# zhaobinglei/REGNet_for_3D_Grasping

Measured on AMD Instinct MI355X. Metric: scenes/sec (25 600-pt ScoreNet+GRN fwd), higher is better.
Workload: dtype f32; 1 GPU; configs[2]: ScoreNet+GraspRegionNet+RefineNet forward, 25600-pt synthetic scenes, batch=8 per GPU, eval; points=25600, batch_per_gpu=8, global_batch=8, parallelism=scene-sharded x1 (no data-path collective), sampling_group_batches=8, sampling_lookahead_batches=32, distinct_batches=8, region_head=synthetic.calibrate_region_head on batch 0, geometry_pending_at_enqueue=9, hip_graphs=False

## Files before the change

### include/regnet_hip.h

```cpp
#ifndef REGNET_HIP_H_
#define REGNET_HIP_H_

#include <stdint.h>

#ifdef __cplusplus
extern "C" {
#endif

#define REGNET_OK 0
#define REGNET_ERR_SHAPE (-1)
#define REGNET_ERR_NULL (-2)
#define REGNET_ERR_UNSUPPORTED (-3)

int regnet_abi_version(void);
const char* regnet_build_info(void);
const char* regnet_strerror(int code);

int regnet_fps_f32(const float* xyz, int64_t sb, int64_t sc, int64_t sn, int64_t B, int64_t N,
                   int64_t M, int64_t* index, float* workspace, void* stream);
int64_t regnet_fps_workspace_bytes(int64_t B, int64_t N, int64_t M);
int regnet_fps_chain_f32(const float* xyz, int64_t sb, int64_t sc, int64_t sn, int64_t B, int64_t N, int64_t M,
                         int64_t* index, float* workspace, const int32_t* prefix_ok, int32_t* first_tie, void* stream);
int64_t regnet_fps_status_offset_bytes(int64_t B, int64_t N, int64_t M);
int regnet_fps_plan(int64_t B, int64_t N, int64_t M, int64_t* plan);

int regnet_ball_query_f32(const float* xyz, int64_t sb, int64_t sc, int64_t sn,
                          const float* centroids, int64_t cb, int64_t cc, int64_t cn, int64_t B,
                          int64_t N1, int64_t N2, float radius, int64_t K, int64_t* index,
                          int64_t* count, void* stream);

int64_t regnet_grid_workspace_bytes(int64_t B, int64_t N_source);
int regnet_three_nn_grid_f32(const float* query, int64_t qb, int64_t qc, int64_t qn, const float* key,
                             int64_t kb, int64_t kc, int64_t kn, int64_t B, int64_t N1, int64_t N2,
                             int64_t* index, float* dist2, void* workspace, void* stream);
int regnet_ball_query_grid_f32(const float* xyz, int64_t sb, int64_t sc, int64_t sn,
                               const float* centroids, int64_t cb, int64_t cc, int64_t cn, int64_t B,
                               int64_t N1, int64_t N2, float radius, int64_t K, int64_t* index,
                               int64_t* count, void* workspace, void* stream);

int regnet_group_points_fwd_f32(const float* input, int64_t sb, int64_t sc, int64_t sn,
                                const int64_t* index, int64_t B, int64_t C, int64_t N1, int64_t N2,
                                int64_t K, float* out, void* stream);
int regnet_group_points_bwd_f32(const float* grad_out, int64_t sb, int64_t sc, int64_t sn2,
                                int64_t sk, const int64_t* index, int64_t B, int64_t C, int64_t N1,
                                int64_t N2, int64_t K, float* grad_in, void* stream);

int regnet_three_nn_f32(const float* query, int64_t qb, int64_t qc, int64_t qn, const float* key,
                        int64_t kb, int64_t kc, int64_t kn, int64_t B, int64_t N1, int64_t N2,
                        int64_t* index, float* dist2, void* stream);

int regnet_interpolate_fwd_f32(const float* input, int64_t sb, int64_t sc, int64_t sm,
                               const int64_t* index, const float* weight, int64_t B, int64_t C,
                               int64_t M, int64_t N, float* out, void* stream);
int regnet_interpolate_bwd_f32(const float* grad_out, int64_t sb, int64_t sc, int64_t sn,
                               const int64_t* index, const float* weight, int64_t B, int64_t C,
                               int64_t M, int64_t N, float* grad_in, void* stream);

int regnet_gather_knn_fwd_f32(const float* input, int64_t sb, int64_t sc, int64_t sn,
                              const int64_t* index, int64_t B, int64_t C, int64_t N, int64_t NI,
                              int64_t K, float* out, void* stream);
int regnet_gather_knn_bwd_f32(const float* grad_out, int64_t sb, int64_t sc, int64_t sn2,
                              int64_t sk, const int64_t* index, int64_t B, int64_t C, int64_t N,
                              int64_t NI, int64_t K, float* grad_in, void* stream);

int64_t regnet_fps_f64_workspace_bytes(int64_t B, int64_t N, int64_t M);
int regnet_fps_f64(const double* xyz, int64_t sb, int64_t sc, int64_t sn, int64_t B, int64_t N, int64_t M,
                   int64_t* index, double* workspace, void* stream);
int regnet_ball_query_f64(const double* xyz, int64_t sb, int64_t sc, int64_t sn, const double* centroids, int64_t cb,
                          int64_t cc, int64_t cn, int64_t B, int64_t N1, int64_t N2, float radius, int64_t K,
                          int64_t* index, int64_t* count, void* stream);
int regnet_three_nn_f64(const double* query, int64_t qb, int64_t qc, int64_t qn, const double* key, int64_t kb,
                        int64_t kc, int64_t kn, int64_t B, int64_t N1, int64_t N2, int64_t* index, double* dist2,
                        void* stream);
int64_t regnet_scatter_f64_workspace_bytes(int64_t B, int64_t num_dest, int64_t num_src);
int regnet_group_points_fwd_f64(const double* input, int64_t sb, int64_t sc, int64_t sn, const int64_t* index, int64_t B,
                                int64_t C, int64_t N1, int64_t N2, int64_t K, double* out, void* stream);
int regnet_group_points_bwd_f64(const double* grad_out, int64_t sb, int64_t sc, int64_t sn2, int64_t sk,
                                const int64_t* index, int64_t B, int64_t C, int64_t N1, int64_t N2, int64_t K,
                                double* grad_in, void* workspace, void* stream);
int regnet_interpolate_fwd_f64(const double* input, int64_t sb, int64_t sc, int64_t sm, const int64_t* index,
                               const double* weight, int64_t B, int64_t C, int64_t M, int64_t N, double* out,
                               void* stream);
int regnet_interpolate_bwd_f64(const double* grad_out, int64_t sb, int64_t sc, int64_t sn, const int64_t* index,
                               const double* weight, int64_t B, int64_t C, int64_t M, int64_t N, double* grad_in,
                               void* workspace, void* stream);
int regnet_gather_knn_fwd_f64(const double* input, int64_t sb, int64_t sc, int64_t sn, const int64_t* index, int64_t B,
                              int64_t C, int64_t N, int64_t NI, int64_t K, double* out, void* stream);
int regnet_gather_knn_bwd_f64(const double* grad_out, int64_t sb, int64_t sc, int64_t sn2, int64_t sk,
                              const int64_t* index, int64_t B, int64_t C, int64_t N, int64_t NI, int64_t K,
                              double* grad_in, void* workspace, void* stream);

int regnet_radius_group_f32(const float* pc, int64_t pb, int64_t pn, const float* centres,
                            int64_t cb, int64_t cn, int64_t B, int64_t N, int64_t NC,
                            float d2_threshold, int64_t cap, int32_t* cand, int32_t* count,
                            void* stream);

int regnet_select_positive_f32(const float* pc, int64_t pb, int64_t pn, const float* score, int64_t sb,
                               int64_t B, int64_t N, float threshold, int64_t* index, float* xyz_out,
                               int32_t* count, void* stream);

int regnet_box_crop_f32(const float* group_points, int64_t gb, int64_t gn, const float* centre,
                        const float* rot, const float* xlim, const float* ylim, float zlim,
                        int64_t n, int64_t G, int32_t* cand, int32_t* count, void* stream);

int regnet_gather_max_f32(const float* feat, int64_t num_rows, int64_t F, const int64_t* rows,
                          int64_t R, int64_t G, float* out, void* stream);
int regnet_gather_max_scene_f32(const float* feat, int64_t num_rows, int64_t F, const int64_t* rows, const int64_t* row_ids,
                                int64_t R, int64_t G, int64_t per_scene, int64_t scene_stride, float* out, void* stream);

int regnet_mlp_layer_f32(const float* A, int64_t lda, int64_t Ka, const float* W, int64_t Kpad,
                         const float* scale, const float* shift, float* C, int64_t ldc, int64_t P,
                         int64_t N, int relu, int pool_group, void* stream);

int64_t regnet_mlp_splitk_workspace_bytes(int64_t P, int64_t N, int64_t ksplit);
int regnet_mlp_layer_splitk_f32(const float* A, int64_t lda, int64_t Ka, const float* W, int64_t Kpad,
                                const float* scale, const float* shift, float* C, int64_t ldc, int64_t P,
                                int64_t N, int relu, int64_t ksplit, void* workspace, void* stream);

int regnet_mlp_layer_plan(int64_t P, int64_t N, int64_t Kpad, int pool_group, int64_t* plan);

int regnet_sa_layer1_f32(const float* feat, int64_t fb, int64_t fn, int64_t fc, int64_t Cf,
                         const float* xyz, int64_t xb, int64_t xc, int64_t xn, const int64_t* nbr,
                         const int64_t* ctr, int64_t B, int64_t M, int64_t group, const float* W,
                         int64_t Kpad, const float* scale, const float* shift, float* C, int64_t ldc,
                         int64_t N, int relu, void* stream);

int regnet_sa_layer12_f32(const float* feat, int64_t fb, int64_t fn, int64_t fc, int64_t Cf,
                          const float* xyz, int64_t xb, int64_t xc, int64_t xn, const int64_t* nbr,
// ... 339 lines not shown
```

### regnet_for_3d_grasping_amd/csrc/build.py

```python
import hashlib
import os
import subprocess
import sys

HERE = os.path.dirname(os.path.abspath(__file__))
OUT = os.path.join(HERE, "libregnet_hip.so")
ARCH = "gfx950"

SOURCES = [
    ("api.hip", []),
    ("geometry.hip", ["-ffp-contract=off", "-fno-slp-vectorize"]),
    ("gather.hip", []),
    ("region.hip", ["-ffp-contract=off"]),
    ("grid.hip", ["-ffp-contract=off"]),
    ("mlp.hip", []),
    ("sa_chain.hip", ["-fno-slp-vectorize"]),
    ("rowchain.hip", ["-fno-slp-vectorize"]),
    ("heads.hip", []),
    ("heads_train.hip", []),
    ("losses.hip", ["-ffp-contract=off"]),
    ("tgemm.hip", []),
    ("sa_split.hip", ["-fno-slp-vectorize"]),
    ("tsplit.hip", []),
    ("bn_train.hip", []),
# ... 10 lines not shown
    ("cluster.hip", ["-ffp-contract=off"]),
    ("fuse.hip", ["-ffp-contract=off"]),
    ("icp.hip", ["-ffp-contract=off"]),
    ("approach.hip", ["-ffp-contract=off"]),
    ("outlier.hip", ["-ffp-contract=off"]),
    ("tsdf.hip", ["-ffp-contract=off"]),
]
COMMON = ["--offload-arch=" + ARCH, "-O3", "-std=c++17", "-fPIC", "-Wall", "-Wno-unused-function",
          "-fno-gpu-rdc"]


def _hipcc():
    for cand in (os.environ.get("HIPCC"), "/opt/rocm/bin/hipcc", "hipcc"):
        if cand and (os.path.isabs(cand) and os.path.exists(cand) or not os.path.isabs(cand)):
            return cand
    raise RuntimeError("hipcc not found")


def _stamp():
    h = hashlib.sha256()
    for name in sorted(os.listdir(HERE)):
        if name.endswith((".hip", ".h", ".py")):
            with open(os.path.join(HERE, name), "rb") as f:
                h.update(name.encode()); h.update(f.read())
    inc = os.path.join(HERE, "..", "..", "include", "regnet_hip.h")
    with open(inc, "rb") as f:
        h.update(f.read())
    return h.hexdigest()


REPO = os.path.dirname(os.path.dirname(HERE))
NO_VGPR_SPILL = {"mlp.o": ["mlp_gemm_kernelILi0E", "gemm2_kernel"], "sa_chain.o": ["sa_chain_kernel"],
                 "rowchain.o": ["sa_premul_chain_kernel", "sa3_premul_chain_kernel", "fp_head_chain_kernelILb0E"],
                 "heads.o": ["heads_chain_kernel", "heads_tree_kernel"], "ops_f64.o": ["_f64_kernel"],
                 "scatter.o": ["scatter_", "segsum_"], "det.o": ["det_"],
                 "ingest.o": ["ingest_"], "nms.o": ["nms_"], "plane.o": ["plane_"], "depth.o": ["depth_"],
                 "fuse.o": ["fuse_"], "icp.o": ["icp_"], "outlier.o": ["outlier_"], "tsdf.o": ["tsdf_"]}


def check_no_vgpr_spill(obj_path, fragments):
    import shutil
    import tempfile
    llvm = "/opt/rocm/lib/llvm/bin"
    objdump, readelf = os.path.join(llvm, "llvm-objdump"), os.path.join(llvm, "llvm-readelf")
    if not (os.path.exists(objdump) and os.path.exists(readelf)):
        return None
    tmp = tempfile.mkdtemp(prefix="regnet_co_")
    try:
        local = os.path.join(tmp, os.path.basename(obj_path))
        shutil.copy(obj_path, local)
        subprocess.run([objdump, "--offloading", local], cwd=tmp, stdout=subprocess.DEVNULL, stderr=subprocess.DEVNULL)
        found = 0
        for name in os.listdir(tmp):
            if "amdgcn" not in name:
                continue
            notes = subprocess.run([readelf, "--notes", os.path.join(tmp, name)], stdout=subprocess.PIPE, stderr=subprocess.DEVNULL).stdout.decode()
            kernel = None
            for line in notes.splitlines():
                line = line.strip()
                if line.startswith(".name:"):
                    kernel = line.split(":", 1)[1].strip()
                elif line.startswith(".vgpr_spill_count:") and kernel and any(f in kernel for f in fragments):
                    found += 1
                    if int(line.split(":", 1)[1]) != 0:
                        raise RuntimeError("%s: %s spills %s vector registers" % (os.path.basename(obj_path), kernel, line.split(":", 1)[1].strip()))
        return found
# ... 78 lines not shown
```

### regnet_for_3d_grasping_amd/csrc/grid.hip

```cpp
#include "grid.h"

__device__ __forceinline__ void nn3_insert(float d, int j, float& d0, float& d1, float& d2, int& i0, int& i1,
                                           int& i2) {
  const bool b2 = d < d2 || (d == d2 && j < i2);
  if (!b2) return;
  const bool b1 = d < d1 || (d == d1 && j < i1);
  const bool b0 = d < d0 || (d == d0 && j < i0);
  d2 = b1 ? d1 : d;
  i2 = b1 ? i1 : j;
  d1 = b0 ? d0 : (b1 ? d : d1);
  i1 = b0 ? i0 : (b1 ? j : i1);
  d0 = b0 ? d : d0;
  i0 = b0 ? j : i0;
}

__global__ __launch_bounds__(256) void three_nn_grid_kernel(const float* __restrict__ query, int64_t qb, int64_t qc,
                                                            int64_t qn, int N1, const char* __restrict__ ws,
                                                            long long slab, int64_t* __restrict__ index,
                                                            float* __restrict__ dist2) {
  const int b = blockIdx.y;
  const int i = blockIdx.x * 256 + threadIdx.x;
  if (i >= N1) return;
  char* my = const_cast<char*>(ws) + (long long)b * slab;
  const GridHeader H = *reinterpret_cast<const GridHeader*>(my);
// ... 292 lines not shown
      }
    }
  }
  int m = 0;
  if (A[1][1] < A[m][m]) m = 1;
  if (A[2][2] < A[m][m]) m = 2;
  n[0] = m == 0 ? V[0][0] : (m == 1 ? V[0][1] : V[0][2]);
  n[1] = m == 0 ? V[1][0] : (m == 1 ? V[1][1] : V[1][2]);
  n[2] = m == 0 ? V[2][0] : (m == 1 ? V[2][1] : V[2][2]);
}

__global__ __launch_bounds__(256) void normal_eigen_kernel(const float* __restrict__ xyz, int N,
                                                           const double* __restrict__ cov, const int* __restrict__ count,
                                                           double cx, double cy, double cz, float* __restrict__ normals) {
  const int i = blockIdx.x * 256 + threadIdx.x;
  if (i >= N) return;
  double n[3] = {0., 0., 1.};
  if (count[i] >= 3) {
    sym3_min_eigenvector(cov + (int64_t)i * 6, n);
    if (n[0] == 0. && n[1] == 0. && n[2] == 0.) { n[2] = 1.; }
  }
  double len = sqrt(n[0] * n[0] + n[1] * n[1] + n[2] * n[2]);
  if (len > 0.) { n[0] /= len; n[1] /= len; n[2] /= len; }
  const double rx = cx - (double)xyz[(int64_t)i * 3], ry = cy - (double)xyz[(int64_t)i * 3 + 1],
               rz = cz - (double)xyz[(int64_t)i * 3 + 2];
  if (n[0] * rx + n[1] * ry + n[2] * rz < 0.) { n[0] = -n[0]; n[1] = -n[1]; n[2] = -n[2]; }
  normals[(int64_t)i * 3] = (float)n[0];
  normals[(int64_t)i * 3 + 1] = (float)n[1];
  normals[(int64_t)i * 3 + 2] = (float)n[2];
}

extern "C" int64_t regnet_grid_workspace_bytes(int64_t B, int64_t N) { return B * grid_slab_bytes(N); }

extern "C" int regnet_three_nn_grid_f32(const float* query, int64_t qb, int64_t qc, int64_t qn, const float* key,
                                        int64_t kb, int64_t kc, int64_t kn, int64_t B, int64_t N1, int64_t N2,
                                        int64_t* index, float* dist2, void* workspace, void* stream) {
  if (N2 < 3 || B < 0 || N1 < 0) return REGNET_ERR_SHAPE;
  if (N1 >= (int64_t)1 << 31 || N2 >= (int64_t)1 << 31 || B > 65535) return REGNET_ERR_UNSUPPORTED;
  if (B == 0 || N1 == 0) return REGNET_OK;
  if (!query || !key || !index || !dist2 || !workspace) return REGNET_ERR_NULL;
  hipStream_t st = as_stream(stream);
  int rc = build_grid(key, kb, kc, kn, B, N2, 0.f, workspace, st);
  if (rc) return rc;
  dim3 grid((unsigned)((N1 + 255) / 256), (unsigned)B);
  hipLaunchKernelGGL(three_nn_grid_kernel, grid, dim3(256), 0, st, query, qb, qc, qn, (int)N1, (const char*)workspace,
                     grid_slab_bytes(N2), index, dist2);
  REGNET_LAUNCH_CHECK();
  return REGNET_OK;
}

extern "C" int regnet_ball_query_grid_f32(const float* xyz, int64_t sb, int64_t sc, int64_t sn, const float* centroids,
                                          int64_t cb, int64_t cc, int64_t cn, int64_t B, int64_t N1, int64_t N2,
                                          float radius, int64_t K, int64_t* index, int64_t* count, void* workspace,
                                          void* stream) {
  if (K <= 0 || B < 0 || N1 < 0 || N2 < 0) return REGNET_ERR_SHAPE;
  if (K > 64 || !(radius > 0.f) || N1 >= (int64_t)1 << 31 || N2 >= (int64_t)1 << 31 || B > 65535)
    return REGNET_ERR_UNSUPPORTED;
  if (B == 0 || N2 == 0) return REGNET_OK;
  if (!centroids || !index || !count || !workspace || (N1 > 0 && !xyz)) return REGNET_ERR_NULL;
  hipStream_t st = as_stream(stream);
  int rc = build_grid(xyz, sb, sc, sn, B, N1, radius, workspace, st);
  if (rc) return rc;
  const float r2 = radius * radius;
  dim3 grid((unsigned)((N2 + 3) / 4), (unsigned)B);
  hipLaunchKernelGGL(ball_query_grid_kernel, grid, dim3(256), 0, st, centroids, cb, cc, cn, (int)N2, r2, radius, (int)K,
                     (const char*)workspace, grid_slab_bytes(N1), index, count);
// ... 31 lines not shown
```

### regnet_for_3d_grasping_amd/csrc/region.hip

```cpp
#include "common.h"

#define RG_WAVES 4

#define RG_UNROLL 4
__device__ __forceinline__ unsigned long long rg_hits(const float* __restrict__ p, int64_t pn, int j, int end,
                                                      float cx, float cy, float cz, float thr) {
  bool hit = false;
  if (j < end) {
    const float* r = p + (int64_t)j * pn;
    hit = sqdist3(r[0], r[1], r[2], cx, cy, cz) <= thr;
  }
  return __ballot(hit);
}

__global__ __launch_bounds__(RG_WAVES * 64) void radius_group_kernel(
    const float* __restrict__ pc, int64_t pb, int64_t pn, const float* __restrict__ ctr, int64_t cb, int64_t cn,
    int N, int NC, float thr, int64_t cap, int32_t* __restrict__ cand, int32_t* __restrict__ count) {
  __shared__ int wave_cnt[RG_WAVES];
  const int lane = threadIdx.x & 63, wave = threadIdx.x >> 6;
  const int c = blockIdx.x;
  const int b = blockIdx.y;
  const float* p = pc + (int64_t)b * pb;
  const float* q = ctr + (int64_t)b * cb + (int64_t)c * cn;
  const float cx = q[0], cy = q[1], cz = q[2];
  int32_t* out = cand + ((int64_t)b * NC + c) * cap;
  const unsigned long long lt_mask = (1ull << lane) - 1ull;
  const int per = ((N + RG_WAVES - 1) / RG_WAVES + 63) / 64 * 64;
  const int beg = min(N, wave * per), end = min(N, beg + per);
  int cnt = 0;
  for (int j0 = beg; j0 < end; j0 += 64 * RG_UNROLL) {
    unsigned long long m[RG_UNROLL];
#pragma unroll
    for (int u = 0; u < RG_UNROLL; ++u) m[u] = rg_hits(p, pn, j0 + 64 * u + lane, end, cx, cy, cz, thr);
#pragma unroll
    for (int u = 0; u < RG_UNROLL; ++u) cnt += (int)__popcll(m[u]);
  }
  if (lane == 0) wave_cnt[wave] = cnt;
  __syncthreads();
  int base = 0, total = 0;
#pragma unroll
  for (int w = 0; w < RG_WAVES; ++w) {
    const int v = wave_cnt[w];
    base += w < wave ? v : 0;
    total += v;
  }
  if (threadIdx.x == 0) count[(int64_t)b * NC + c] = total;
  if (cnt == 0 || base >= cap) return;
  for (int j0 = beg; j0 < end; j0 += 64 * RG_UNROLL) {
    unsigned long long m[RG_UNROLL];
#pragma unroll
    for (int u = 0; u < RG_UNROLL; ++u) m[u] = rg_hits(p, pn, j0 + 64 * u + lane, end, cx, cy, cz, thr);
#pragma unroll
    for (int u = 0; u < RG_UNROLL; ++u) {
      if ((m[u] >> lane) & 1ull) {
        const int pos = base + (int)__popcll(m[u] & lt_mask);
        if (pos < cap) out[pos] = j0 + 64 * u + lane;
      }
      base += (int)__popcll(m[u]);
    }
  }
}

extern "C" int regnet_radius_group_f32(const float* pc, int64_t pb, int64_t pn, const float* centres, int64_t cb,
                                       int64_t cn, int64_t B, int64_t N, int64_t NC, float d2_threshold,
                                       int64_t cap, int32_t* cand, int32_t* count, void* stream) {
  if (B < 0 || N < 0 || NC < 0 || cap < 0) return REGNET_ERR_SHAPE;
  if (N >= (int64_t)1 << 31 || B > 65535) return REGNET_ERR_UNSUPPORTED;
  if (B == 0 || NC == 0) return REGNET_OK;
  if (!centres || !count || (cap > 0 && !cand) || (N > 0 && !pc)) return REGNET_ERR_NULL;
  if (NC >= (int64_t)1 << 31) return REGNET_ERR_UNSUPPORTED;
  dim3 grid((unsigned)NC, (unsigned)B);
  hipLaunchKernelGGL(radius_group_kernel, grid, dim3(RG_WAVES * 64), 0, as_stream(stream), pc, pb, pn, centres, cb,
                     cn, (int)N, (int)NC, d2_threshold, cap, cand, count);
  REGNET_LAUNCH_CHECK();
  return REGNET_OK;
}

#define SP_WAVES 8
__global__ __launch_bounds__(SP_WAVES * 64) void select_positive_kernel(const float* __restrict__ pc, int64_t pb, int64_t pn,
                                                                       const float* __restrict__ score, int64_t sb, int N,
                                                                       float thr, int64_t* __restrict__ index,
                                                                       float* __restrict__ xyz_out, int32_t* __restrict__ count) {
  __shared__ int wave_cnt[SP_WAVES];
  const int tid = threadIdx.x, lane = tid & 63;
  const int wave = __builtin_amdgcn_readfirstlane(tid >> 6);
  const int b = blockIdx.x;
  const float* p = pc + (int64_t)b * pb;
  const float* sc = score + (int64_t)b * sb;
  int64_t* idx = index + (int64_t)b * N;
  float* xo = xyz_out + (int64_t)b * 3 * N;
  const unsigned long long lt_mask = (1ull << lane) - 1ull;
  const int seg = ((N + SP_WAVES - 1) / SP_WAVES + 63) / 64 * 64;
  const int lo = wave * seg, hi = lo + seg < N ? lo + seg : N;
// ... 610 lines not shown
```

### regnet_for_3d_grasping_amd/fused.py

```python
import collections
import ctypes

import torch

from . import _lib, pn2_ext

ENABLED = True
CHAIN3 = True
SPLITK_MAX_ROWS = 1024
PREMUL = True
PREMUL_CENTRE = True
ROWCHAIN = True
SA3_CHAIN = True
FP_HEAD_INTERP = True

SaRoute = collections.namedtuple("SaRoute", "features tail prepare")


def sa_route(module, has_feature=True):
    mlp, n = module.mlp, len(module.mlp)
    if getattr(module.grouper, "num_neighbours", 0) != 64 or n < 2 or (has_feature and not module.use_xyz):
        return None
    width = [block.conv.out_channels for block in mlp]
    relu = [block.relu is not None for block in mlp]
# ... 419 lines not shown
    "sa_layer1": lambda feature, xyz, nbr, ctr, layer, B, M, group: _flop_meta(B * M * group, layer.K, layer.N),
    "sa_premul_layer": lambda U, V, nbr, layer, B, Nsrc, M, group, pool_group=0:
        _flop_meta(B * M * group, layer.K, layer.N),
    "sa_chain3": lambda feature, xyz, nbr, ctr, l1, l2, l3, B, M, group, count=None, order=None:
        "P%d K%d N%d flop%d" % (B * M * group, l3.K, l3.N,
                                2 * B * M * group * (l1.K * l1.N + l2.K * l2.N + l3.K * l3.N)),
    "sa_premul_chain": lambda U, V, nbr, module, layers, B, Nsrc, M:
        "P%d K256 N512 flop%d" % (B * M * 64, 2 * B * M * 64 * (256 * 256 + 256 * 512)),
    "sa3_premul_chain": lambda U, V, nbr, module, layers, B, Nsrc, M:
        "P%d K512 N1024 flop%d" % (B * M * 64, 2 * B * M * 64 * (512 * 512 + 512 * 1024)),
    "fp_head_chain_interp": lambda Ys, idx, dist2, eps, dense_small, wd4, first, seg, fp_layers, B, Ns, Nd:
        "P%d K256 N256 flop%d" % (B * Nd, 2 * B * Nd * 491520),
    "fp_head_chain": lambda h1, seg, fp_layers, P: "P%d K256 N256 flop%d" % (P, 2 * P * 491520),
    "sa_layer12": lambda feature, xyz, nbr, ctr, first, layer, B, M, group, pool_group=0:
        "P%d K%d N%d flop%d" % (B * M * group, layer.K, layer.N,
                                2 * B * M * group * (layer.K * layer.N + first.K * first.N)),
}


def _as_channels_last(feature):
    cl = feature.transpose(1, 2)
    return cl if cl.is_contiguous() else cl.contiguous()


def sa_sample(module, xyz, prefix_ok=None):
    chain = pn2_ext.FpsChain(prefix_ok if FPS_CHAIN else None)
    ctr = pn2_ext.farthest_point_sample(xyz, module.num_centroids, chain)
    return ctr, chain.first_tie


def sa_group(module, xyz, ctr, first_tie=None):
    B, M = ctr.shape
    new_xyz = pn2_ext.gather_points(xyz, ctr) if xyz.dtype == torch.float32 else torch.gather(xyz, 2, ctr[:, None, :].expand(B, 3, M))
    nbr, count = pn2_ext.ball_query(xyz, new_xyz, module.grouper.radius, module.grouper.num_neighbours)
    geo = {"ctr": ctr, "new_xyz": new_xyz, "nbr": nbr}
    if first_tie is not None:
        geo["first_tie"] = first_tie
    route = sa_route(module)
    prepare = route.prepare if route is not None else None
    if prepare == "pairs":
        geo["count"] = count
        geo["order"] = chain3_pair_order(count)
    elif prepare == "premul":
        _, (_, v_layer) = _sa_packs(module, route, module.mlp[0].conv.in_channels - 3, xyz.device)
        geo.update(_premul_centres(xyz, new_xyz, v_layer))
    return geo


def sa_geometry(module, xyz, ctr=None, prefix_ok=None):
    if ctr is not None:
        return sa_group(module, xyz, ctr)
    ctr, first_tie = sa_sample(module, xyz, prefix_ok)
    return sa_group(module, xyz, ctr, first_tie)


def sa_features(module, xyz, feature, geo):
    B, N1 = xyz.shape[0], xyz.shape[2]
    M, K = module.num_centroids, module.grouper.num_neighbours
    Cf = 0 if feature is None else feature.size(1)
    route = sa_route(module, feature is not None)
    if route is None:
        raise NotImplementedError("fused SA supports 64 neighbours, >= 2 MLP layers and features only with use_xyz")
    layers, premul = _sa_packs(module, route, Cf, xyz.device)
    P = B * M * K
    pool = 0 if route.tail else K
    nbr, ctr = geo["nbr"], geo["ctr"]
    if premul is not None:
        u_layer, v_layer = premul
# ... 388 lines not shown
```

### regnet_for_3d_grasping_amd/get_regiondataset.py

```python
import numpy as np
import torch

from . import host_io, np_random, region_ops
from .pn2_utils import function as _F


def get_grasp_allobj(pc, predict_score, params, data_paths, use_theta=True, defer_large_groups=False):
    (center_num, score_thre, group_num, r_time_group, group_num_more, r_time_group_more,
     width, height, depth) = params
    center_pc, center_pc_index = _select_score_center(pc, predict_score, center_num, score_thre)
    labels_pending = None
    if pc.is_cuda and (DEVICE_DRAWS or (pc.shape[0] * pc.shape[1] > BATCHED_SEARCH_MAX_POINTS and len(data_paths) == 0)):
        pc_group_index, pc_group = _get_group_pc(pc, center_pc, center_pc_index, group_num, width, height, depth,
                                                 r_time_group)
        pc_group_more_index, pc_group_more = _get_group_pc(pc, center_pc, center_pc_index, group_num_more, width,
                                                           height, depth, r_time_group_more)
    else:
        cand_s, count_s = region_ops.radius_candidates(pc, center_pc, group_radius(width, height, depth, r_time_group))
        cand_m, count_m = region_ops.radius_candidates(pc, center_pc, group_radius(width, height, depth, r_time_group_more))
        if len(data_paths) > 0 and pc.is_cuda:
            labels_pending = _get_center_grasp(center_pc_index, center_pc, data_paths, depth, use_theta, defer_read=True)
        np_random.flush()
        counts = torch.stack((count_s, count_m)).cpu().numpy()
        def drawn(count, size):
            if pc.is_cuda:
                return np_random.choice_rows_pinned(count, size, 0)[0].to(pc.device, non_blocking=True)
            return host_io.upload(np_random.choice_rows(count, size, 0)[0], pc.device)

        pos = drawn(counts[0], group_num)
        pc_group_index, pc_group = region_ops.resample_groups(pc, cand_s, pos)

        def large_groups():
            return region_ops.resample_groups(pc, cand_m, drawn(counts[1], group_num_more))

        if defer_large_groups and DEFER_LARGE_GROUPS and pc.is_cuda:
            pc_group_more_index, pc_group_more = large_groups, None
        else:
            pc_group_more_index, pc_group_more = large_groups()
    grasp_labels = None
    if labels_pending is not None:
        grasp_labels = labels_pending() if callable(labels_pending) else labels_pending
    elif len(data_paths) > 0:
        grasp_labels = _get_center_grasp(center_pc_index, center_pc, data_paths, depth, use_theta)
    np_random.flush_unless_deferred()
    return center_pc, center_pc_index, pc_group_index, pc_group, pc_group_more_index, pc_group_more, grasp_labels


DEFER_LARGE_GROUPS = True
LABEL_KERNEL = True
BATCHED_LABELS = True
NO_GRASP_SQ_DISTANCE = 0.005

# ... 163 lines not shown
            np_random.flush()
            extra = np.random.choice(P, center_num - P, replace=True)
            local = torch.cat([torch.arange(P), torch.from_numpy(np.asarray(extra, dtype=np.int64))])
            index[b] = map_index[local.to(pc.device)]
        else:
            np_random.flush()
            picks = np.random.choice(N, center_num, replace=False)
            index[b] = host_io.upload(np.asarray(picks, dtype=np.int64), pc.device)
    if pc.is_cuda and pc.dtype == torch.float32:
        from . import pn2_ext
        center_pc = pn2_ext.gather_points(pc.transpose(1, 2), index, channels_last=True)
    else:
        center_pc = torch.gather(pc, 1, index.unsqueeze(-1).expand(B, center_num, C))
    return center_pc, index


def group_radius(width, height, depth, r_time):
    return float(np.float32(max(width, height, depth) * r_time))


DEVICE_DRAWS = False
BATCHED_SEARCH_MAX_POINTS = 4 * 25600


def _draw_positions(counts, group_num, max_count):
    if DEVICE_DRAWS and counts.is_cuda:
        return np_random.choice_rows_device(counts.int(), group_num, 0, max_count)[0]
    np_random.flush()
    if counts.is_cuda:
        return np_random.choice_rows_pinned(counts.cpu().numpy(), group_num, 0)[0].to(counts.device, non_blocking=True)
    return host_io.upload(np_random.choice_rows(counts.cpu().numpy(), group_num, 0)[0], counts.device)


def _get_group_pc(pc, center_pc, center_pc_index, group_num, width, height, depth, r_time):
    B, N, C = pc.shape
    Nc = center_pc.shape[1]
    radius = group_radius(width, height, depth, r_time)
    cand, counts = region_ops.radius_candidates(pc, center_pc, radius)
    pos = _draw_positions(counts, group_num, N)
    pc_group_index, pc_group = region_ops.resample_groups(pc, cand, pos)
    return pc_group_index, pc_group
```

### regnet_for_3d_grasping_amd/pipeline.py

```python
import contextlib
import io

import torch

from . import synthetic
from .get_regiondataset import get_grasp_allobj
from .gripper_region_network import GripperRegionNetwork
from .score_network import ScoreNetwork

CENTER_NUM, SCORE_THRE = 64, 0.5
GROUP_NUM, R_TIME_GROUP = 256, 0.1
GROUP_NUM_MORE, R_TIME_GROUP_MORE = 1024, 0.8
WIDTH, HEIGHT, DEPTH = 0.08, 0.01, 0.06
GRIPPER_NUM, GRASP_SCORE_THRESHOLD, REG_CHANNEL = 64, 0.5, 10

PARAMS = [CENTER_NUM, SCORE_THRE, GROUP_NUM, R_TIME_GROUP, GROUP_NUM_MORE, R_TIME_GROUP_MORE, WIDTH, HEIGHT, DEPTH]
GRIPPER_PARAMS = [WIDTH, HEIGHT, DEPTH]


def build_models(device, score_seed=7, region_seed=11):
    score_net = ScoreNetwork(training=True)
    score_net.load_state_dict(synthetic.seeded_state_dict(score_net, score_seed))
    region_net = GripperRegionNetwork(training=True, group_num=GROUP_NUM, gripper_num=GRIPPER_NUM,
                                      grasp_score_threshold=GRASP_SCORE_THRESHOLD, radius=DEPTH,
# ... 260 lines not shown
    def _wants_graphs(self, pc):
        want = self.graphs
        if want == "auto":
            want = pc.shape[0] * pc.shape[1] <= GRAPH_MAX_POINTS
        from . import fused
        return bool(want) and fused.ENABLED and len(self.s_mlps) == 1 and not self.score_net.training and pc.is_cuda

    def _features(self, item):
        if "slot" in item:
            return self._features_replay(item)
        s_mlp = self.s_mlps[self._n_featured % len(self.s_mlps)]
        self._n_featured += 1
        from . import fused
        prev = self.__dict__.get("_last_mlp_done")
        if prev is not None and prev.query():
            self.host_late_feature_stages = self.__dict__.get("host_late_feature_stages", 0) + 1
        geo_pending = not item["geo_done"].query()
        if geo_pending:
            self.geometry_pending_at_enqueue = self.__dict__.get("geometry_pending_at_enqueue", 0) + 1
        with torch.cuda.stream(s_mlp), torch.no_grad():
            s_mlp.wait_event(item["geo_done"])
            fused.TAIL_SINK = tails = [] if self.split_chain_tail else None
            try:
                all_feature, score, _ = self.score_net(item["pc"], plan=item["plan"])
            finally:
                fused.TAIL_SINK = None
            done = torch.cuda.Event()
            done.record(s_mlp)
            self._last_mlp_done = done
            item["tail_done"] = list(tails or ())
        all_feature.record_stream(self.s_reg)
        score.record_stream(self.s_reg)
        item.update(all_feature=all_feature, score=score, mlp_done=done)
        item.pop("plan")
        item.pop("ctr")
        return item

    def _region(self, item):
        pc, all_feature, score = item["pc"], item["all_feature"], item["score"]
        out = {"all_feature": all_feature, "score": score}
        with torch.cuda.stream(self.s_reg), torch.no_grad():
            self.s_reg.wait_event(item["mlp_done"])
            for ev in item.get("tail_done", ()):
                self.s_reg.wait_event(ev)
            if self.with_region:
                (center_pc, center_idx, g_idx, g, gm_idx, gm, _) = get_grasp_allobj(pc, score, PARAMS, [])
                with contextlib.redirect_stdout(io.StringIO()):
                    res = self.region_net(g, gm, g_idx, gm_idx, center_pc, center_idx, pc, all_feature,
                                          GRIPPER_PARAMS, None, [])
                out.update(center_pc_index=center_idx, pc_group_index=g_idx, pc_group_more_index=gm_idx,
                           next_grasp=res[0], keep_per_scene=res[1], true_mask=res[2], select_grasp_class=res[6],
                           select_grasp_score=res[7], final_mask=res[11],
                           valid_crops=getattr(self.region_net, "last_valid_crops", None))
            done = torch.cuda.Event()
            done.record(self.s_reg)
        if not self.with_region:
            item["mlp_done"].synchronize()
            for ev in item.get("tail_done", ()):
                ev.synchronize()
        out["done"] = done
        return out

    def run(self, batches, max_pending_regions=3):
        import queue
        import threading

        from . import fused
        cur = torch.cuda.current_stream(self.device)
        with torch.no_grad():
            fused.prepack(self.score_net, self.region_net)
        self._graph_sig = _graph_signature(self.score_net)
        if self._stage_graphs is not None and self._stage_graphs.signature != self._graph_sig:
            self._stage_graphs = None
        streams = tuple(self.s_fps) + tuple(self.s_mlps) + (self.s_geo, self.s_reg)
        for s in streams:
            s.wait_stream(cur)

        todo, done = queue.Queue(), queue.Queue()

# ... 101 lines not shown
```

### regnet_for_3d_grasping_amd/pn2_ext.py

```python
import torch

from . import _lib, determinism

_call = _lib.call
_L = _lib.lib

GRID_MIN_POINTS = 2048
GRID_MIN_POINTS_BALL = 8192


def _need_gpu(t, name):
    if not isinstance(t, torch.Tensor):
        raise TypeError("%s must be a torch.Tensor" % name)
    if not t.is_cuda:
        raise RuntimeError("%s must be a CUDA tensor" % name)


def _need_f32(t, name):
    _need_gpu(t, name)
    if t.dtype != torch.float32:
        raise RuntimeError("%s must be float32 (REGNet's path is fp32 only)" % name)


def _need_float(t, name, like=None):
    _need_gpu(t, name)
    if t.dtype not in (torch.float32, torch.float64):
        raise RuntimeError("%s must be float32 or float64" % name)
    if like is not None and t.dtype != like.dtype:
        raise RuntimeError("%s is %s but the other float inputs are %s" % (name, t.dtype, like.dtype))
    return t.dtype == torch.float64


# ... 81 lines not shown
    _call("regnet_class_order_i64", count, flat.data_ptr(), flat.numel(), order.data_ptr())
    return order


def pair_order(count):
    _need_i64(count, "count")
    flat = count.reshape(-1)
    flat = flat if flat.is_contiguous() else flat.contiguous()
    order = torch.empty((flat.numel(),), dtype=torch.int64, device=count.device)
    work = torch.empty((flat.numel(),), dtype=torch.int32, device=count.device)
    _call("regnet_pair_order_i64", count, flat.data_ptr(), flat.numel(), order.data_ptr(), work.data_ptr())
    return order


_fps_flags = {}


def _fps_flag(device):
    key = (device.type, device.index if device.index is not None else torch.cuda.current_device())
    if key not in _fps_flags:
        _fps_flags[key] = torch.zeros(1, dtype=torch.int32, device=device)
    return _fps_flags[key]


def raise_if_fps_failed():
    for flag in _fps_flags.values():
        if int(flag.item()):
            flag.zero_()
            raise RuntimeError("farthest_point_sample: a cooperating workgroup lost its partner (launch not fully "
                               "resident?) -- the returned indices are incomplete -- or gather_points saw an index "
                               "outside the cloud")


def ball_query(points, centroids, radius, num_neighbours):
    f64 = _need_float(points, "points")
    _need_float(centroids, "centroids", points)
    _eq(points.size(1), 3, "points.size(1) does not equal to 3")
    _eq(centroids.size(1), 3, "centroids.size(1) does not equal to 3")
    _eq(centroids.size(0), points.size(0), "centroids.size(0) does not equal to batch_size")
    B, _, N1 = points.shape
    N2 = centroids.size(2)
    K = int(num_neighbours)
    index = torch.empty((B, N2, K), dtype=torch.int64, device=points.device)
    count = torch.empty((B, N2), dtype=torch.int64, device=points.device)
    if not f64 and N1 >= GRID_MIN_POINTS_BALL and K <= 64 and B > 0 and float(radius) > 0:
        ws = torch.empty((_L.regnet_grid_workspace_bytes(B, N1),), dtype=torch.uint8, device=points.device)
        _call("regnet_ball_query_grid_f32", points, points.data_ptr(), *points.stride(), centroids.data_ptr(),
              *centroids.stride(), B, N1, N2, float(radius), K, index.data_ptr(), count.data_ptr(), ws.data_ptr())
    else:
        _call(_entry("ball_query", points), points, points.data_ptr(), *points.stride(), centroids.data_ptr(),
              *centroids.stride(), B, N1, N2, float(radius), K, index.data_ptr(), count.data_ptr())
    return [index, count]


def group_points_forward(input, index):
    _need_float(input, "input")
    _need_i64(index, "index")
    _eq(input.dim(), 3, "input.dim() does not equal to 3")
    _eq(index.dim(), 3, "index.dim() does not equal to 3")
    _eq(index.size(0), input.size(0), "index.size(0) does not equal to batch_size")
    B, C, N1 = input.shape
    _, N2, K = index.shape
    idx = index.contiguous()
    out = torch.empty((B, C, N2, K), dtype=input.dtype, device=input.device)
    _call(_entry("group_points_fwd", input), input, input.data_ptr(), *input.stride(), idx.data_ptr(), B, C, N1, N2, K,
          out.data_ptr())
    return out


def group_points_backward(grad_output, index, num_points, plan=None):
    _need_float(grad_output, "grad_output")
    _need_i64(index, "index")
    _eq(grad_output.dim(), 4, "grad_output.dim() does not equal to 4")
    _eq(index.dim(), 3, "index.dim() does not equal to 3")
    B, C, N2, K = grad_output.shape
    _eq(index.size(0), B, "index.size(0) does not equal to batch_size")
    _eq(index.size(1), N2, "index.size(1) does not equal to num_select")
    _eq(index.size(2), K, "index.size(2) does not equal to k")
    N1 = int(num_points)
    idx = index.contiguous()
    return _scatter_backward(
# ... 115 lines not shown
```

### regnet_for_3d_grasping_amd/region_ops.py

```python
import numpy as np
import torch

from . import _lib, determinism
from .pn2_ext import _need_f32, _need_i64

_call = _lib.call


def sqrt_le_threshold(radius):
    r = np.float32(radius)
    if not r >= 0:
        return float("-inf")
    t = np.float32(np.float64(r) * np.float64(r))
    inf = np.float32(np.inf)
    while np.sqrt(t) > r:
        t = np.nextafter(t, -inf, dtype=np.float32)
    while np.sqrt(np.nextafter(t, inf, dtype=np.float32)) <= r:
        t = np.nextafter(t, inf, dtype=np.float32)
    return float(t)


def radius_candidates(pc, centres, radius):
    _need_f32(pc, "pc")
    _need_f32(centres, "centres")
    if pc.stride(2) != 1 or centres.stride(2) != 1:
        pc, centres = pc.contiguous(), centres.contiguous()
    B, N, _ = pc.shape
    Nc = centres.shape[1]
    cand = torch.empty((B, Nc, max(N, 1)), dtype=torch.int32, device=pc.device)
    count = torch.empty((B, Nc), dtype=torch.int32, device=pc.device)
    _call("regnet_radius_group_f32", pc, pc.data_ptr(), pc.stride(0), pc.stride(1), centres.data_ptr(), centres.stride(0),
          centres.stride(1), B, N, Nc, sqrt_le_threshold(radius), cand.size(2), cand.data_ptr(), count.data_ptr())
    return cand, count


def select_positive(pc, score, threshold):
    _need_f32(pc, "pc")
    _need_f32(score, "score")
    if pc.stride(2) != 1:
        pc = pc.contiguous()
    if score.stride(1) != 1:
        score = score.contiguous()
    B, N, _ = pc.shape
    index = torch.empty((B, max(N, 1)), dtype=torch.int64, device=pc.device)
    xyz = torch.empty((B, 3, max(N, 1)), dtype=torch.float32, device=pc.device)
    count = torch.empty((B,), dtype=torch.int32, device=pc.device)
    _call("regnet_select_positive_f32", pc, pc.data_ptr(), pc.stride(0), pc.stride(1), score.data_ptr(), score.stride(0), B,
          N, float(threshold), index.data_ptr(), xyz.data_ptr(), count.data_ptr())
    return index, xyz, count


def resample_groups(pc, cand, pos):
    _need_f32(pc, "pc")
    _need_i64(pos, "pos")
    if cand.dtype != torch.int32:
        raise TypeError("cand must be int32")
    if pc.stride(2) != 1:
        pc = pc.contiguous()
    cand, pos = cand.contiguous(), pos.contiguous()
    B, Nc, G = pos.shape
    C = pc.shape[2]
    index = torch.empty((B, Nc, G), dtype=torch.int64, device=pc.device)
    points = torch.empty((B, Nc, G, C), dtype=torch.float32, device=pc.device)
    flag = _range_flag(pc.device)
    _call("regnet_resample_groups_f32", pc, pc.data_ptr(), pc.stride(0), pc.stride(1), C, cand.data_ptr(), cand.size(2),
          pos.data_ptr(), B, Nc, G, pc.shape[1], flag.data_ptr(), index.data_ptr(), points.data_ptr())
# ... 200 lines not shown
```

Measured before the change: 1064 scenes/s.

## Reuse SA1 ball-query cell grid for fused two-radius region grouping

Keeps the spatial cell grid built during the first set-abstraction ball query and passes it through the pipeline to the region-grouping stage. A new kernel walks only the grid cells near each centre, testing both the small and large radius in one pass, then bitonic-sorts the hits so the output keeps the original index order. This replaces two exhaustive scans over all points per centre. If a centre's neighbourhood is too large for the shared-memory list, the kernel falls back to the exhaustive scan. The cost is a bitonic sort in shared memory and keeping the grid buffer alive across streams.

Result: no change. 1063 scenes/s, median of 2 (-0.1%).

```diff
diff --git a/include/regnet_hip.h b/include/regnet_hip.h
--- a/include/regnet_hip.h
+++ b/include/regnet_hip.h
@@ -37,6 +37,8 @@
                                const float* centroids, int64_t cb, int64_t cc, int64_t cn, int64_t B,
                                int64_t N1, int64_t N2, float radius, int64_t K, int64_t* index,
                                int64_t* count, void* workspace, void* stream);
+int regnet_grid_build_f32(const float* xyz, int64_t sb, int64_t sc, int64_t sn, int64_t B, int64_t N,
+                          float cell, void* workspace, void* stream);
 
 int regnet_group_points_fwd_f32(const float* input, int64_t sb, int64_t sc, int64_t sn,
                                 const int64_t* index, int64_t B, int64_t C, int64_t N1, int64_t N2,
@@ -94,6 +96,11 @@
                             int64_t cb, int64_t cn, int64_t B, int64_t N, int64_t NC,
                             float d2_threshold, int64_t cap, int32_t* cand, int32_t* count,
                             void* stream);
+int regnet_radius_group2_grid_f32(const float* pc, int64_t pb, int64_t pn, const float* centres,
+                                  int64_t cb, int64_t cn, int64_t B, int64_t N, int64_t NC,
+                                  const void* grid, float T_small, float T_large, int64_t cap_small,
+                                  int64_t cap_large, int32_t* cand_small, int32_t* count_small,
+                                  int32_t* cand_large, int32_t* count_large, void* stream);
 
 int regnet_select_positive_f32(const float* pc, int64_t pb, int64_t pn, const float* score, int64_t sb,
                                int64_t B, int64_t N, float threshold, int64_t* index, float* xyz_out,
diff --git a/regnet_for_3d_grasping_amd/csrc/build.py b/regnet_for_3d_grasping_amd/csrc/build.py
--- a/regnet_for_3d_grasping_amd/csrc/build.py
+++ b/regnet_for_3d_grasping_amd/csrc/build.py
@@ -66,6 +66,7 @@
 REPO = os.path.dirname(os.path.dirname(HERE))
 NO_VGPR_SPILL = {"mlp.o": ["mlp_gemm_kernelILi0E", "gemm2_kernel"], "sa_chain.o": ["sa_chain_kernel"],
                  "rowchain.o": ["sa_premul_chain_kernel", "sa3_premul_chain_kernel", "fp_head_chain_kernelILb0E"],
+                 "region.o": ["radius_group2_grid_kernel"],
                  "heads.o": ["heads_chain_kernel", "heads_tree_kernel"], "ops_f64.o": ["_f64_kernel"],
                  "scatter.o": ["scatter_", "segsum_"], "det.o": ["det_"],
                  "ingest.o": ["ingest_"], "nms.o": ["nms_"], "plane.o": ["plane_"], "depth.o": ["depth_"],
diff --git a/regnet_for_3d_grasping_amd/csrc/grid.hip b/regnet_for_3d_grasping_amd/csrc/grid.hip
--- a/regnet_for_3d_grasping_amd/csrc/grid.hip
+++ b/regnet_for_3d_grasping_amd/csrc/grid.hip
@@ -348,6 +348,15 @@
 
 extern "C" int64_t regnet_grid_workspace_bytes(int64_t B, int64_t N) { return B * grid_slab_bytes(N); }
 
+extern "C" int regnet_grid_build_f32(const float* xyz, int64_t sb, int64_t sc, int64_t sn, int64_t B, int64_t N, float cell,
+                                     void* workspace, void* stream) {
+  if (B < 0 || N < 0 || cell != cell) return REGNET_ERR_SHAPE;
+  if (N >= (int64_t)1 << 31 || B > 65535) return REGNET_ERR_UNSUPPORTED;
+  if (B == 0) return REGNET_OK;
+  if (!workspace || (N > 0 && !xyz)) return REGNET_ERR_NULL;
+  return build_grid(xyz, sb, sc, sn, B, N, cell, workspace, as_stream(stream));
+}
+
 extern "C" int regnet_three_nn_grid_f32(const float* query, int64_t qb, int64_t qc, int64_t qn, const float* key,
                                         int64_t kb, int64_t kc, int64_t kn, int64_t B, int64_t N1, int64_t N2,
                                         int64_t* index, float* dist2, void* workspace, void* stream) {
diff --git a/regnet_for_3d_grasping_amd/csrc/region.hip b/regnet_for_3d_grasping_amd/csrc/region.hip
--- a/regnet_for_3d_grasping_amd/csrc/region.hip
+++ b/regnet_for_3d_grasping_amd/csrc/region.hip
@@ -1,4 +1,4 @@
-#include "common.h"
+#include "grid.h"
 
 #define RG_WAVES 4
 
@@ -13,17 +13,10 @@
   return __ballot(hit);
 }
 
-__global__ __launch_bounds__(RG_WAVES * 64) void radius_group_kernel(
-    const float* __restrict__ pc, int64_t pb, int64_t pn, const float* __restrict__ ctr, int64_t cb, int64_t cn,
-    int N, int NC, float thr, int64_t cap, int32_t* __restrict__ cand, int32_t* __restrict__ count) {
-  __shared__ int wave_cnt[RG_WAVES];
+__device__ __forceinline__ void rg_exhaustive(const float* __restrict__ p, int64_t pn, int N, float cx, float cy, float cz,
+                                              float thr, int64_t cap, int32_t* __restrict__ out,
+                                              int32_t* __restrict__ count_out, int* wave_cnt) {
   const int lane = threadIdx.x & 63, wave = threadIdx.x >> 6;
-  const int c = blockIdx.x;
-  const int b = blockIdx.y;
-  const float* p = pc + (int64_t)b * pb;
-  const float* q = ctr + (int64_t)b * cb + (int64_t)c * cn;
-  const float cx = q[0], cy = q[1], cz = q[2];
-  int32_t* out = cand + ((int64_t)b * NC + c) * cap;
   const unsigned long long lt_mask = (1ull << lane) - 1ull;
   const int per = ((N + RG_WAVES - 1) / RG_WAVES + 63) / 64 * 64;
   const int beg = min(N, wave * per), end = min(N, beg + per);
@@ -44,7 +37,7 @@
     base += w < wave ? v : 0;
     total += v;
   }
-  if (threadIdx.x == 0) count[(int64_t)b * NC + c] = total;
+  if (threadIdx.x == 0) *count_out = total;
   if (cnt == 0 || base >= cap) return;
   for (int j0 = beg; j0 < end; j0 += 64 * RG_UNROLL) {
     unsigned long long m[RG_UNROLL];
@@ -59,6 +52,187 @@
       base += (int)__popcll(m[u]);
     }
   }
+}
+
+__global__ __launch_bounds__(RG_WAVES * 64) void radius_group_kernel(
+    const float* __restrict__ pc, int64_t pb, int64_t pn, const float* __restrict__ ctr, int64_t cb, int64_t cn,
+    int N, int NC, float thr, int64_t cap, int32_t* __restrict__ cand, int32_t* __restrict__ count) {
+  __shared__ int wave_cnt[RG_WAVES];
+  const int c = blockIdx.x;
+  const int b = blockIdx.y;
+  const float* q = ctr + (int64_t)b * cb + (int64_t)c * cn;
+  rg_exhaustive(pc + (int64_t)b * pb, pn, N, q[0], q[1], q[2], thr, cap, cand + ((int64_t)b * NC + c) * cap,
+                count + (int64_t)b * NC + c, wave_cnt);
+}
+
+#define RG2_T (RG_WAVES * 64)
+#define RG2_LIST 4096
+#define RG2_RUNS 512
+
+__global__ __launch_bounds__(RG2_T) void radius_group2_grid_kernel(
+    const float* __restrict__ pc, int64_t pb, int64_t pn, const float* __restrict__ ctr, int64_t cb, int64_t cn, int N, int NC,
+    const char* __restrict__ ws, long long slab, float radius_l, float thr_s, float thr_l, int64_t cap_s, int64_t cap_l,
+    int32_t* __restrict__ cand_s, int32_t* __restrict__ count_s, int32_t* __restrict__ cand_l, int32_t* __restrict__ count_l) {
+  __shared__ unsigned list[RG2_LIST];
+  __shared__ int run_off[RG2_RUNS + 1];
+  __shared__ int run_delta[RG2_RUNS];
+  __shared__ int wave_cnt[2][RG_WAVES];
+  __shared__ int n_large;
+  const int tid = threadIdx.x, lane = tid & 63, wave = tid >> 6;
+  const int c = blockIdx.x;
+  const int b = blockIdx.y;
+  const float* q = ctr + (int64_t)b * cb + (int64_t)c * cn;
+  const float cx = q[0], cy = q[1], cz = q[2];
+  const int64_t oc = (int64_t)b * NC + c;
+  char* my = const_cast<char*>(ws) + (long long)b * slab;
+  const GridHeader H = *reinterpret_cast<const GridHeader*>(my);
+  const int* cell_start = grid_cell_start(my);
+  const float4* sorted = grid_sorted(my);
+  const float pad = radius_l * 1.0001f + H.eps + 4e-6f * fmaxf(fmaxf(fabsf(cx), fabsf(cy)), fabsf(cz));
+  const bool any = thr_l >= 0.f && pad >= 0.f;
+  const int x0 = cell_coord(cx - pad, H.lo[0], H.inv_h, H.dim[0]), x1 = cell_coord(cx + pad, H.lo[0], H.inv_h, H.dim[0]);
+  const int y0 = cell_coord(cy - pad, H.lo[1], H.inv_h, H.dim[1]), y1 = cell_coord(cy + pad, H.lo[1], H.inv_h, H.dim[1]);
+  const int z0 = cell_coord(cz - pad, H.lo[2], H.inv_h, H.dim[2]), z1 = cell_coord(cz + pad, H.lo[2], H.inv_h, H.dim[2]);
+  const int ny = y1 - y0 + 1;
+  const int nruns = any ? ny * (z1 - z0 + 1) : 0;
+  bool walked = nruns <= RG2_RUNS;
+  int mine_s = 0;
+  if (tid == 0) n_large = 0;
+  if (walked) {
+    int len[2], beg[2];
+#pragma unroll
+    for (int u = 0; u < 2; ++u) {
+      const int r = 2 * tid + u;
+      len[u] = beg[u] = 0;
+      if (r < nruns) {
+        const int row = ((z0 + r / ny) * H.dim[1] + (y0 + r % ny)) * H.dim[0];
+        beg[u] = cell_start[row + x0];
+        len[u] = max(cell_start[row + x1 + 1] - beg[u], 0);
+      }
+    }
+    int incl = len[0] + len[1];
+#pragma unroll
+    for (int off = 1; off < 64; off <<= 1) {
+      const int o = __shfl_up(incl, off, 64);
+      if (lane >= off) incl += o;
+    }
+    if (lane == 63) wave_cnt[0][wave] = incl;
+    __syncthreads();
+    int first = incl - (len[0] + len[1]), total = 0;
+#pragma unroll
+    for (int w = 0; w < RG_WAVES; ++w) {
+      const int v = wave_cnt[0][w];
+      first += w < wave ? v : 0;
+      total += v;
+    }
+#pragma unroll
+    for (int u = 0; u < 2; ++u) {
+      const int r = 2 * tid + u;
+      if (r < nruns) { run_off[r] = first; run_delta[r] = beg[u] - first; }
+      first += len[u];
+    }
+    if (tid == 0) run_off[nruns] = total;
+    __syncthreads();
+    for (int k0 = 0; k0 < total; k0 += RG2_T) {
+      const int k = k0 + tid;
+      bool in_l = false, in_s = false;
+      unsigned j = 0u;
+      if (k < total) {
+        int lo = 0, hi = nruns;
+        while (hi - lo > 1) {
+          const int mid = (lo + hi) >> 1;
+          if (run_off[mid] <= k) lo = mid; else hi = mid;
+        }
+        const int slot = k + run_delta[lo];
+        if (slot >= 0 && slot < N) {
+          const float4 p = sorted[slot];
+          const float d2 = sqdist3(p.x, p.y, p.z, cx, cy, cz);
+          in_l = d2 <= thr_l;
+          in_s = in_l && d2 <= thr_s;
+          j = (unsigned)__float_as_int(p.w);
+        }
+      }
+      const int at = wave_append(in_l, &n_large);
+      if (in_l && at < RG2_LIST) list[at] = (j << 1) | (in_s ? 1u : 0u);
+      mine_s += in_s ? 1 : 0;
+    }
+    __syncthreads();
+    walked = n_large <= RG2_LIST;
+  }
+  if (!walked) {
+    const float* p = pc + (int64_t)b * pb;
+    rg_exhaustive(p, pn, N, cx, cy, cz, thr_s, cap_s, cand_s + oc * cap_s, count_s + oc, wave_cnt[0]);
+    rg_exhaustive(p, pn, N, cx, cy, cz, thr_l, cap_l, cand_l + oc * cap_l, count_l + oc, wave_cnt[1]);
+    return;
+  }
+  const int nl = n_large;
+  int P = 2;
+  while (P < nl) P <<= 1;
+  for (int i = nl + tid; i < P; i += RG2_T) list[i] = 0xffffffffu;
+  __syncthreads();
+  for (int k = 2; k <= P && nl > 1; k <<= 1)
+    for (int jj = k >> 1; jj > 0; jj >>= 1) {
+      for (int t = tid; t < (P >> 1); t += RG2_T) {
+        const int i = ((t & ~(jj - 1)) << 1) | (t & (jj - 1)), l = i | jj;
+        const unsigned a = list[i], bb = list[l];
+        if ((a > bb) == ((i & k) == 0)) { list[i] = bb; list[l] = a; }
+      }
+      __syncthreads();
+    }
+#pragma unroll
+  for (int o = 32; o > 0; o >>= 1) mine_s += __shfl_xor(mine_s, o);
+  if (lane == 0) wave_cnt[1][wave] = mine_s;
+  int32_t* out_l = cand_l + oc * cap_l;
+  for (int i = tid; i < nl && i < cap_l; i += RG2_T) out_l[i] = (int32_t)(list[i] >> 1);
+  const int per = ((nl + RG_WAVES - 1) / RG_WAVES + 63) / 64 * 64;
+  const int beg = min(nl, wave * per), end = min(nl, beg + per);
+  int cnt = 0;
+  for (int i0 = beg; i0 < end; i0 += 64) {
+    const int i = i0 + lane;
+    cnt += (int)__popcll(__ballot(i < end && (list[i] & 1u)));
+  }
+  if (lane == 0) wave_cnt[0][wave] = cnt;
+  __syncthreads();
+  int base = 0, ns = 0;
+#pragma unroll
+  for (int w = 0; w < RG_WAVES; ++w) {
+    base += w < wave ? wave_cnt[0][w] : 0;
+    ns += wave_cnt[1][w];
+  }
+  if (tid == 0) { count_l[oc] = nl; count_s[oc] = ns; }
+  int32_t* out_s = cand_s + oc * cap_s;
+  const unsigned long long lt_mask = (1ull << lane) - 1ull;
+  for (int i0 = beg; i0 < end && base < cap_s; i0 += 64) {
+    const int i = i0 + lane;
+    const unsigned key = i < end ? list[i] : 0u;
+    const unsigned long long m = __ballot((key & 1u) != 0u);
+    if (key & 1u) {
+      const int pos = base + (int)__popcll(m & lt_mask);
+      if (pos < cap_s) out_s[pos] = (int32_t)(key >> 1);
+    }
+    base += (int)__popcll(m);
+  }
+}
+
+extern "C" int regnet_radius_group2_grid_f32(const float* pc, int64_t pb, int64_t pn, const float* centres, int64_t cb,
+                                             int64_t cn, int64_t B, int64_t N, int64_t NC, const void* grid, float T_small,
+                                             float T_large, int64_t cap_small, int64_t cap_large, int32_t* cand_small,
+                                             int32_t* count_small, int32_t* cand_large, int32_t* count_large, void* stream) {
+  if (B < 0 || N < 0 || NC < 0 || cap_small < 0 || cap_large < 0) return REGNET_ERR_SHAPE;
+  if (T_small > T_large || T_small != T_small || T_large != T_large) return REGNET_ERR_SHAPE;
+  if (N >= (int64_t)1 << 30 || B > 65535) return REGNET_ERR_UNSUPPORTED;
+  if (B == 0 || NC == 0) return REGNET_OK;
+  if (!centres || !grid || !count_small || !count_large || (cap_small > 0 && !cand_small) || (cap_large > 0 && !cand_large) ||
+      (N > 0 && !pc))
+    return REGNET_ERR_NULL;
+  if (NC >= (int64_t)1 << 31) return REGNET_ERR_UNSUPPORTED;
+  const float radius_l = T_large >= 0.f ? sqrtf(T_large) : -1.f;
+  dim3 launch((unsigned)NC, (unsigned)B);
+  hipLaunchKernelGGL(radius_group2_grid_kernel, launch, dim3(RG2_T), 0, as_stream(stream), pc, pb, pn, centres, cb, cn, (int)N,
+                     (int)NC, (const char*)grid, grid_slab_bytes(N), radius_l, T_small, T_large, cap_small, cap_large, cand_small,
+                     count_small, cand_large, count_large);
+  REGNET_LAUNCH_CHECK();
+  return REGNET_OK;
 }
 
 extern "C" int regnet_radius_group_f32(const float* pc, int64_t pb, int64_t pn, const float* centres, int64_t cb,
diff --git a/regnet_for_3d_grasping_amd/fused.py b/regnet_for_3d_grasping_amd/fused.py
--- a/regnet_for_3d_grasping_amd/fused.py
+++ b/regnet_for_3d_grasping_amd/fused.py
@@ -475,8 +475,11 @@
 def sa_group(module, xyz, ctr, first_tie=None):
     B, M = ctr.shape
     new_xyz = pn2_ext.gather_points(xyz, ctr) if xyz.dtype == torch.float32 else torch.gather(xyz, 2, ctr[:, None, :].expand(B, 3, M))
-    nbr, count = pn2_ext.ball_query(xyz, new_xyz, module.grouper.radius, module.grouper.num_neighbours)
+    with pn2_ext.kept_grids() as grids:
+        nbr, count = pn2_ext.ball_query(xyz, new_xyz, module.grouper.radius, module.grouper.num_neighbours)
     geo = {"ctr": ctr, "new_xyz": new_xyz, "nbr": nbr}
+    if grids:
+        geo["grid"] = grids[0]
     if first_tie is not None:
         geo["first_tie"] = first_tie
     route = sa_route(module)
diff --git a/regnet_for_3d_grasping_amd/get_regiondataset.py b/regnet_for_3d_grasping_amd/get_regiondataset.py
--- a/regnet_for_3d_grasping_amd/get_regiondataset.py
+++ b/regnet_for_3d_grasping_amd/get_regiondataset.py
@@ -5,19 +5,30 @@
 from .pn2_utils import function as _F
 
 
-def get_grasp_allobj(pc, predict_score, params, data_paths, use_theta=True, defer_large_groups=False):
+def get_grasp_allobj(pc, predict_score, params, data_paths, use_theta=True, defer_large_groups=False, grid=None):
     (center_num, score_thre, group_num, r_time_group, group_num_more, r_time_group_more,
      width, height, depth) = params
     center_pc, center_pc_index = _select_score_center(pc, predict_score, center_num, score_thre)
     labels_pending = None
     if pc.is_cuda and (DEVICE_DRAWS or (pc.shape[0] * pc.shape[1] > BATCHED_SEARCH_MAX_POINTS and len(data_paths) == 0)):
+        found = found_more = None
+        if grid is not None and r_time_group <= r_time_group_more:
+            cand_s, count_s, cand_m, count_m = region_ops.radius_candidates2(
+                pc, center_pc, group_radius(width, height, depth, r_time_group),
+                group_radius(width, height, depth, r_time_group_more), grid)
+            found, found_more = (cand_s, count_s), (cand_m, count_m)
         pc_group_index, pc_group = _get_group_pc(pc, center_pc, center_pc_index, group_num, width, height, depth,
-                                                 r_time_group)
+                                                 r_time_group, found)
         pc_group_more_index, pc_group_more = _get_group_pc(pc, center_pc, center_pc_index, group_num_more, width,
-                                                           height, depth, r_time_group_more)
+                                                           height, depth, r_time_group_more, found_more)
     else:
-        cand_s, count_s = region_ops.radius_candidates(pc, center_pc, group_radius(width, height, depth, r_time_group))
-        cand_m, count_m = region_ops.radius_candidates(pc, center_pc, group_radius(width, height, depth, r_time_group_more))
+        if grid is not None and pc.is_cuda and r_time_group <= r_time_group_more:
+            cand_s, count_s, cand_m, count_m = region_ops.radius_candidates2(
+                pc, center_pc, group_radius(width, height, depth, r_time_group),
+                group_radius(width, height, depth, r_time_group_more), grid)
+        else:
+            cand_s, count_s = region_ops.radius_candidates(pc, center_pc, group_radius(width, height, depth, r_time_group))
+            cand_m, count_m = region_ops.radius_candidates(pc, center_pc, group_radius(width, height, depth, r_time_group_more))
         if len(data_paths) > 0 and pc.is_cuda:
             labels_pending = _get_center_grasp(center_pc_index, center_pc, data_paths, depth, use_theta, defer_read=True)
         np_random.flush()
@@ -247,11 +258,11 @@
     return host_io.upload(np_random.choice_rows(counts.cpu().numpy(), group_num, 0)[0], counts.device)
 
 
-def _get_group_pc(pc, center_pc, center_pc_index, group_num, width, height, depth, r_time):
+def _get_group_pc(pc, center_pc, center_pc_index, group_num, width, height, depth, r_time, found=None):
     B, N, C = pc.shape
     Nc = center_pc.shape[1]
     radius = group_radius(width, height, depth, r_time)
-    cand, counts = region_ops.radius_candidates(pc, center_pc, radius)
+    cand, counts = found if found is not None else region_ops.radius_candidates(pc, center_pc, radius)
     pos = _draw_positions(counts, group_num, N)
     pc_group_index, pc_group = region_ops.resample_groups(pc, cand, pos)
     return pc_group_index, pc_group
diff --git a/regnet_for_3d_grasping_amd/pipeline.py b/regnet_for_3d_grasping_amd/pipeline.py
--- a/regnet_for_3d_grasping_amd/pipeline.py
+++ b/regnet_for_3d_grasping_amd/pipeline.py
@@ -316,6 +316,10 @@
         all_feature.record_stream(self.s_reg)
         score.record_stream(self.s_reg)
         item.update(all_feature=all_feature, score=score, mlp_done=done)
+        grid = item["plan"]["sa"][0].get("grid") if self.with_region else None
+        if grid is not None:
+            grid.buffer.record_stream(self.s_reg)
+            item["grid"] = grid
         item.pop("plan")
         item.pop("ctr")
         return item
@@ -328,7 +332,8 @@
             for ev in item.get("tail_done", ()):
                 self.s_reg.wait_event(ev)
             if self.with_region:
-                (center_pc, center_idx, g_idx, g, gm_idx, gm, _) = get_grasp_allobj(pc, score, PARAMS, [])
+                (center_pc, center_idx, g_idx, g, gm_idx, gm, _) = get_grasp_allobj(pc, score, PARAMS, [],
+                                                                                    grid=item.get("grid"))
                 with contextlib.redirect_stdout(io.StringIO()):
                     res = self.region_net(g, gm, g_idx, gm_idx, center_pc, center_idx, pc, all_feature,
                                           GRIPPER_PARAMS, None, [])
diff --git a/regnet_for_3d_grasping_amd/pn2_ext.py b/regnet_for_3d_grasping_amd/pn2_ext.py
--- a/regnet_for_3d_grasping_amd/pn2_ext.py
+++ b/regnet_for_3d_grasping_amd/pn2_ext.py
@@ -1,3 +1,7 @@
+import collections
+import contextlib
+import threading
+
 import torch
 
 from . import _lib, determinism
@@ -145,6 +149,31 @@
                                "outside the cloud")
 
 
+class CellGrid(collections.namedtuple("CellGrid", "buffer batch num_points")):
+    __slots__ = ()
+
+
+def build_grid(points, cell=0.0):
+    _need_f32(points, "points")
+    _eq(points.size(1), 3, "points.size(1) does not equal to 3")
+    B, _, N = points.shape
+    ws = torch.empty((max(_L.regnet_grid_workspace_bytes(B, N), 1),), dtype=torch.uint8, device=points.device)
+    _call("regnet_grid_build_f32", points, points.data_ptr(), *points.stride(), B, N, float(cell), ws.data_ptr())
+    return CellGrid(ws, B, N)
+
+
+_kept = threading.local()
+
+
+@contextlib.contextmanager
+def kept_grids():
+    before, _kept.grids = getattr(_kept, "grids", None), []
+    try:
+        yield _kept.grids
+    finally:
+        _kept.grids = before
+
+
 def ball_query(points, centroids, radius, num_neighbours):
     f64 = _need_float(points, "points")
     _need_float(centroids, "centroids", points)
@@ -160,6 +189,8 @@
         ws = torch.empty((_L.regnet_grid_workspace_bytes(B, N1),), dtype=torch.uint8, device=points.device)
         _call("regnet_ball_query_grid_f32", points, points.data_ptr(), *points.stride(), centroids.data_ptr(),
               *centroids.stride(), B, N1, N2, float(radius), K, index.data_ptr(), count.data_ptr(), ws.data_ptr())
+        if N2 > 0 and getattr(_kept, "grids", None) is not None:
+            _kept.grids.append(CellGrid(ws, B, N1))
     else:
         _call(_entry("ball_query", points), points, points.data_ptr(), *points.stride(), centroids.data_ptr(),
               *centroids.stride(), B, N1, N2, float(radius), K, index.data_ptr(), count.data_ptr())
diff --git a/regnet_for_3d_grasping_amd/region_ops.py b/regnet_for_3d_grasping_amd/region_ops.py
--- a/regnet_for_3d_grasping_amd/region_ops.py
+++ b/regnet_for_3d_grasping_amd/region_ops.py
@@ -32,6 +32,26 @@
     _call("regnet_radius_group_f32", pc, pc.data_ptr(), pc.stride(0), pc.stride(1), centres.data_ptr(), centres.stride(0),
           centres.stride(1), B, N, Nc, sqrt_le_threshold(radius), cand.size(2), cand.data_ptr(), count.data_ptr())
     return cand, count
+
+
+def radius_candidates2(pc, centres, radius_small, radius_large, grid=None):
+    if grid is None:
+        return radius_candidates(pc, centres, radius_small) + radius_candidates(pc, centres, radius_large)
+    _need_f32(pc, "pc")
+    _need_f32(centres, "centres")
+    if pc.stride(2) != 1 or centres.stride(2) != 1:
+        pc, centres = pc.contiguous(), centres.contiguous()
+    B, N, _ = pc.shape
+    if (grid.batch, grid.num_points) != (B, N) or grid.buffer.device != pc.device:
+        raise ValueError("radius_candidates2: the grid is of %d x %d points, the cloud of %d x %d" % (
+            grid.batch, grid.num_points, B, N))
+    Nc = centres.shape[1]
+    cand = torch.empty((2, B, Nc, max(N, 1)), dtype=torch.int32, device=pc.device)
+    count = torch.empty((2, B, Nc), dtype=torch.int32, device=pc.device)
+    _call("regnet_radius_group2_grid_f32", pc, pc.data_ptr(), pc.stride(0), pc.stride(1), centres.data_ptr(), centres.stride(0),
+          centres.stride(1), B, N, Nc, grid.buffer.data_ptr(), sqrt_le_threshold(radius_small), sqrt_le_threshold(radius_large),
+          cand.size(3), cand.size(3), cand[0].data_ptr(), count[0].data_ptr(), cand[1].data_ptr(), count[1].data_ptr())
+    return cand[0], count[0], cand[1], count[1]
 
 
 def select_positive(pc, score, threshold):
```
